# testingautomated-usi/simple-tip

Measured on AMD Instinct MI355X. Metric: inputs_per_sec_prioritized, higher is better.
Workload: dtype bf16; 1 GPU; model=cifar10_resnet20, global_batch=20480, parallelism=dp1, train_ats=50000, at_width=4096, input_residency=hbm, scorers=gini+softmax-family+dsa+pc-lsa

## Files before the change

### simple_tip_amd/ops/hip/bindings.cpp

```cpp

#include <torch/extension.h>

#include <ATen/hip/HIPContext.h>
#include <c10/hip/HIPStream.h>
#include <hip/hip_runtime.h>

#include <vector>

void launch_rownorm(const float*, int, int, float*, hipStream_t);
void launch_pairwise_full(const float*, const float*, const float*,
                          const float*, int, int, int, float*, hipStream_t);
void launch_pairwise_rowmin(const float*, const float*, const float*,
                            const float*, int, int, int, float*, int*, float*,
                            int64_t*, hipStream_t);
void launch_pairwise_kde(const float*, const float*, const float*,
                         const float*, int, int, int, float2*, float*,
                         hipStream_t);
void launch_grouped_rowmin(const float*, const float*, const float*,
                           const float*, const int*, const int*, int, int,
                           int, int, float*, int*, float*, int64_t*,
                           hipStream_t);
void launch_grouped_kde(const float*, const float*, const float*,
                        const float*, const int*, const int*, int, int, int,
                        int, float2*, float*, hipStream_t);
void launch_grouped_rowmin_bf16(const short*, const short*, const float*,
                                const float*, const int*, const int*, int,
                                int, int, int, float*, int*, float*,
                                int64_t*, hipStream_t);
void launch_grouped_kde_bf16(const short*, const short*, const float*,
                             const float*, const int*, const int*, int, int,
                             int, int, float2*, float*, hipStream_t);
void launch_profile(int, const float*, const unsigned char*, const float*,
                    const float*, float, int, int, int, int,
                    unsigned long long*, long long*, hipStream_t);
void launch_popcount(const unsigned long long*, int, int, long long*,
                     hipStream_t);
void launch_tknc(const float*, int, int, int, int, int, unsigned long long*,
                 hipStream_t);
void launch_bucketize(const double*, const double*, int, int, int,
                      unsigned long long*, hipStream_t);
void launch_cam_greedy_coop(const unsigned long long*, int, int,
                            unsigned long long, unsigned char*,
                            unsigned long long*, long long*, int*, long long*,
                            int*, int*, int*, hipStream_t);
void launch_softmax_scores(const float*, int, int, float*, float*, float*,
                           float*, hipStream_t);
void launch_mfma_probe(const short*, const short*, float*, hipStream_t);
void launch_resblock(int, int, const short*, short*, const short*,
                     const float*, const short*, const float*, hipStream_t);
void launch_downblock(int, int, const short*, short*, const short*,
                      const float*, const short*, const float*, const short*,
                      const float*, hipStream_t);
void launch_stem(int, const short*, short*, const short*, const float*,
                 hipStream_t);
void launch_stage1(int, const float*, short*, const void* const*, hipStream_t);
void launch_stage2(int, const short*, short*, const void* const*, hipStream_t);
void launch_stage3(int, const short*, short*, float*, const void* const*,
                   hipStream_t);
void launch_mc_dropout_votes(const float*, const float*, const float*, int,
                             int, int, int, uint32_t, float, uint32_t,
                             uint32_t, uint32_t, int*, hipStream_t);
void launch_mc_dropout_stats(const float*, const float*, const float*, int,
                             int, int, int, uint32_t, float, uint32_t,
                             uint32_t, uint32_t, int*, float*, float*,
                             hipStream_t);
int segment_plan_max_classes();
void launch_segment_plan(const int64_t*, int, int, int, int*, int*, int*,
                         hipStream_t);
void launch_rownorm_bf16(const short*, int, int, const int*, float*,
                         hipStream_t);
int grouped_whiten_max_features();
void launch_grouped_whiten_bf16(const short*, int, int, const int*, const int*,
                                const int*, int, const int*, const short*, int,
                                int, int, int, short*, hipStream_t);
void launch_grouped_rowmin_plan(const short*, int, const short*, const float*,
                                const float*, const int*, const int*,
                                const int*, const float*, int, int, int, int,
                                float*, int*, float*, float*, int*,
                                hipStream_t);
void launch_grouped_kde_plan(const short*, const short*, const float*,
                             const float*, const int*, const int*, const int*,
                             int, const int*, const float*, int, int, int, int,
                             float2*, float*, hipStream_t);
void launch_grouped_center(const void*, bool, int, int, const int*, const int*,
                           const int*, int, int, const float*, int, float*,
                           hipStream_t);
int grouped_gauss_max_slots();
void launch_grouped_gauss_plan(const float*, const float*, const int*,
                               const int*, const int*, int, const float*, int,
                               int, int, int, float*, float*, hipStream_t);
int mc_dropout_max_grid(int, int);
int mc_dropout_rows_per_block();
int mc_dropout_max_classes();
int mc_dropout_max_features();

namespace {

hipStream_t cur_stream() {
  return c10::hip::getCurrentHIPStream().stream();
}

void check_f32_2d(const torch::Tensor& t, const char* name) {
  TORCH_CHECK(t.is_cuda(), name, " must be on GPU");
  TORCH_CHECK(t.dtype() == torch::kFloat32, name, " must be fp32");
  TORCH_CHECK(t.dim() == 2 && t.is_contiguous(), name,
              " must be 2D contiguous");
}

constexpr int kBN = 128;

torch::Tensor rownorm(torch::Tensor x) {
  check_f32_2d(x, "x");
  auto out = torch::empty({x.size(0)}, x.options());
  launch_rownorm(x.data_ptr<float>(), x.size(0), x.size(1),
                 out.data_ptr<float>(), cur_stream());
  return out;
}

torch::Tensor pairwise_sqdist(torch::Tensor a, torch::Tensor b) {
  check_f32_2d(a, "a");
  check_f32_2d(b, "b");
  TORCH_CHECK(a.size(1) == b.size(1), "feature dims differ");
  const int m = a.size(0), n = b.size(0), k = a.size(1);
  auto an = rownorm(a);
  auto bn = rownorm(b);
  auto out = torch::empty({m, n}, a.options());
  launch_pairwise_full(a.data_ptr<float>(), b.data_ptr<float>(),
                       an.data_ptr<float>(), bn.data_ptr<float>(), m, n, k,
                       out.data_ptr<float>(), cur_stream());
  return out;
}

std::vector<torch::Tensor> rowmin_l2(torch::Tensor a, torch::Tensor b,
                                     c10::optional<torch::Tensor> bnorm) {
  check_f32_2d(a, "a");
  check_f32_2d(b, "b");
  TORCH_CHECK(a.size(1) == b.size(1), "feature dims differ");
  TORCH_CHECK(b.size(0) > 0, "rowmin_l2 against empty set");
  const int m = a.size(0), n = b.size(0), k = a.size(1);
  const int jb = (n + kBN - 1) / kBN;
  auto an = rownorm(a);
  auto bn = bnorm.has_value() ? bnorm.value() : rownorm(b);
  auto pval = torch::empty({jb, m}, a.options());
  auto pidx = torch::empty({jb, m}, a.options().dtype(torch::kInt32));
  auto dist = torch::empty({m}, a.options());
  auto idx = torch::empty({m}, a.options().dtype(torch::kInt64));
  launch_pairwise_rowmin(a.data_ptr<float>(), b.data_ptr<float>(),
                         an.data_ptr<float>(), bn.data_ptr<float>(), m, n, k,
                         pval.data_ptr<float>(), pidx.data_ptr<int>(),
                         dist.data_ptr<float>(), idx.data_ptr<int64_t>(),
                         cur_stream());
  return {dist, idx};
}

std::vector<torch::Tensor> grouped_rowmin(
    torch::Tensor testS, torch::Tensor trainS, torch::Tensor tseg,
    torch::Tensor nseg, torch::Tensor bnorm, int64_t jb_max) {
  check_f32_2d(testS, "testS");
  check_f32_2d(trainS, "trainS");
  TORCH_CHECK(tseg.is_cuda() && tseg.dtype() == torch::kInt32);
  TORCH_CHECK(nseg.is_cuda() && nseg.dtype() == torch::kInt32);
  const int bp = testS.size(0), k = testS.size(1);
  const int nclasses = tseg.size(0) - 1;
  auto an = rownorm(testS);
  auto pval = torch::empty({jb_max, bp}, testS.options());
  auto pidx = torch::empty({jb_max, bp}, testS.options().dtype(torch::kInt32));
  auto dist = torch::empty({bp}, testS.options());
  auto idx = torch::empty({bp}, testS.options().dtype(torch::kInt64));
  launch_grouped_rowmin(
      testS.data_ptr<float>(), trainS.data_ptr<float>(), an.data_ptr<float>(),
      bnorm.data_ptr<float>(), tseg.data_ptr<int>(), nseg.data_ptr<int>(),
      nclasses, bp, k, jb_max, pval.data_ptr<float>(), pidx.data_ptr<int>(),
      dist.data_ptr<float>(), idx.data_ptr<int64_t>(), cur_stream());
  return {dist, idx};
}

torch::Tensor grouped_kde(torch::Tensor testWS, torch::Tensor trainWS,
                          torch::Tensor tseg, torch::Tensor nseg,
                          torch::Tensor bnorm, int64_t jb_max) {
  check_f32_2d(testWS, "testWS");
  check_f32_2d(trainWS, "trainWS");
  const int bp = testWS.size(0), k = testWS.size(1);
  const int nclasses = tseg.size(0) - 1;
  auto an = rownorm(testWS);
// ... 497 lines not shown
    const torch::Tensor& b = take();
    TORCH_CHECK(b.is_cuda() && b.dtype() == torch::kFloat32 &&
                    b.is_contiguous() && b.numel() == n,
                "fp32 stage parameter has the wrong type or size");
    ptrs.push_back(b.data_ptr<float>());
  }
  void res(int64_t c) {
    conv(9 * c, c);
    conv(9 * c, c);
  }
  void down(int64_t c) {
    conv(9 * c, 2 * c);
    conv(18 * c, 2 * c);
    conv(c, 2 * c);
  }
  const void* const* done() {
    TORCH_CHECK(next == t.size(), "too many stage parameters");
    return ptrs.data();
  }
};

void check_plane(const torch::Tensor& x, int64_t elems) {
  TORCH_CHECK(x.dim() == 2 && x.size(1) == elems, "x must be [B, ", elems, "]");
}

torch::Tensor resnet_stage1(torch::Tensor x,
                            std::vector<torch::Tensor> params) {
  TORCH_CHECK(x.is_cuda() && x.dtype() == torch::kFloat32 &&
                  x.is_contiguous() && x.dim() == 4 && x.size(1) == 32 &&
                  x.size(2) == 32 && x.size(3) == 3,
              "x must be a contiguous fp32 [B, 32, 32, 3] GPU tensor");
  TORCH_CHECK(reinterpret_cast<uintptr_t>(x.data_ptr()) % 16 == 0,
              "x must be 16-byte aligned");
  StageParams p(params);
  p.conv(9 * 8, 16);
  for (int i = 0; i < 3; ++i) p.res(16);
  p.down(16);
  const void* const* ptrs = p.done();
  const int batch = x.size(0);
  auto out = torch::empty({batch, 16 * 16 * 32},
                          x.options().dtype(torch::kBFloat16));
  if (batch > 0)
    launch_stage1(batch, x.data_ptr<float>(),
                  const_cast<short*>(bf16_ptr(out)), ptrs, cur_stream());
  return out;
}

torch::Tensor resnet_stage2(torch::Tensor x,
                            std::vector<torch::Tensor> params) {
  check_plane(x, 16 * 16 * 32);
  StageParams p(params);
  for (int i = 0; i < 2; ++i) p.res(32);
  p.down(32);
  const void* const* ptrs = p.done();
  const int batch = x.size(0);
  auto out = torch::empty({batch, 8 * 8 * 64}, x.options());
  if (batch > 0)
    launch_stage2(batch, bf16_ptr(x), const_cast<short*>(bf16_ptr(out)), ptrs,
                  cur_stream());
  return out;
}

std::vector<torch::Tensor> resnet_stage3(torch::Tensor x,
                                         std::vector<torch::Tensor> params) {
  check_plane(x, 8 * 8 * 64);
  StageParams p(params);
  for (int i = 0; i < 2; ++i) p.res(64);
  p.f32(10 * 64);
  p.f32(10);
  const void* const* ptrs = p.done();
  const int batch = x.size(0);
  auto ats = torch::empty_like(x);
  auto logits = torch::empty({batch, 10}, x.options().dtype(torch::kFloat32));
  if (batch > 0)
    launch_stage3(batch, bf16_ptr(x), const_cast<short*>(bf16_ptr(ats)),
                  logits.data_ptr<float>(), ptrs, cur_stream());
  return {ats, logits};
}


static void mc_dropout_check(const torch::Tensor& feats,
                             const torch::Tensor& weight,
                             const torch::Tensor& bias, int64_t thresh,
                             int64_t num_samples, int64_t row_offset) {
  check_f32_2d(feats, "feats");
  check_f32_2d(weight, "weight");
  TORCH_CHECK(bias.is_cuda() && bias.dtype() == torch::kFloat32 &&
                  bias.dim() == 1 && bias.is_contiguous(),
              "bias must be a contiguous 1D fp32 GPU tensor");
  const int64_t n = feats.size(0), d = feats.size(1), c = weight.size(0);
  TORCH_CHECK(weight.size(1) == d, "weight must be [C, D]");
  TORCH_CHECK(bias.size(0) == c, "bias must be [C]");
  TORCH_CHECK(c >= 1 && c <= mc_dropout_max_classes() && d >= 1 &&
                  d <= mc_dropout_max_features(),
              "mc_dropout_votes envelope is C <= ", mc_dropout_max_classes(),
              ", D <= ", mc_dropout_max_features());
  TORCH_CHECK(num_samples >= 1 && num_samples <= 65535, "bad num_samples");
  TORCH_CHECK(thresh >= 0 && thresh <= 0xFFFFFFFFll, "bad threshold");
  TORCH_CHECK(n <= 0x7FFFFFFFll && row_offset >= 0 &&
                  row_offset + n <= 0x100000000ll,
              "rows must satisfy row_offset + N <= 2^32");
}

torch::Tensor mc_dropout_votes(torch::Tensor feats, torch::Tensor weight,
                               torch::Tensor bias, int64_t thresh,
                               double scale, int64_t num_samples,
                               int64_t seed_lo, int64_t seed_hi,
                               int64_t row_offset) {
  mc_dropout_check(feats, weight, bias, thresh, num_samples, row_offset);
  const int64_t n = feats.size(0), d = feats.size(1), c = weight.size(0);
  auto votes = torch::empty({n, c}, feats.options().dtype(torch::kInt32));
  if (n == 0) return votes;
  launch_mc_dropout_votes(
      feats.data_ptr<float>(), weight.data_ptr<float>(),
      bias.data_ptr<float>(), (int)n, (int)d, (int)c, (int)num_samples,
      (uint32_t)thresh, (float)scale, (uint32_t)seed_lo, (uint32_t)seed_hi,
      (uint32_t)row_offset, votes.data_ptr<int>(), cur_stream());
  return votes;
}

std::vector<torch::Tensor> mc_dropout_stats(
    torch::Tensor feats, torch::Tensor weight, torch::Tensor bias,
    int64_t thresh, double scale, int64_t num_samples, int64_t seed_lo,
    int64_t seed_hi, int64_t row_offset) {
  mc_dropout_check(feats, weight, bias, thresh, num_samples, row_offset);
  const int64_t n = feats.size(0), d = feats.size(1), c = weight.size(0);
  auto votes = torch::empty({n, c}, feats.options().dtype(torch::kInt32));
  auto mean_probs = torch::empty({n, c}, feats.options());
  auto mean_entropy = torch::empty({n}, feats.options());
  if (n == 0) return {votes, mean_probs, mean_entropy};
  launch_mc_dropout_stats(
      feats.data_ptr<float>(), weight.data_ptr<float>(),
      bias.data_ptr<float>(), (int)n, (int)d, (int)c, (int)num_samples,
      (uint32_t)thresh, (float)scale, (uint32_t)seed_lo, (uint32_t)seed_hi,
      (uint32_t)row_offset, votes.data_ptr<int>(),
      mean_probs.data_ptr<float>(), mean_entropy.data_ptr<float>(),
      cur_stream());
  return {votes, mean_probs, mean_entropy};
}

}

PYBIND11_MODULE(TORCH_EXTENSION_NAME, m) {
  m.doc() = "simple_tip_amd HIP/CDNA4 kernels (gfx950)";
  m.def("rownorm", &rownorm);
  m.def("pairwise_sqdist", &pairwise_sqdist);
  m.def("rowmin_l2", &rowmin_l2, py::arg("a"), py::arg("b"),
        py::arg("bnorm") = py::none());
  m.def("kde_logsumexp", &kde_logsumexp);
  m.def("grouped_rowmin", &grouped_rowmin);
  m.def("grouped_kde", &grouped_kde);
  m.def("grouped_rowmin_bf16", &grouped_rowmin_bf16);
  m.def("grouped_kde_bf16", &grouped_kde_bf16);
  m.def("segment_plan", &segment_plan);
  m.def("segment_plan_out", &segment_plan_out);
  m.def("segment_plan_rows", &segment_plan_rows);
  m.def("rownorm_bf16_out", &rownorm_bf16_out, py::arg("x"), py::arg("out"),
        py::arg("tseg") = py::none());
  m.def("grouped_whiten_bf16", &grouped_whiten_bf16);
  m.def("grouped_whiten_max_features", &grouped_whiten_max_features);
  m.def("grouped_rowmin_plan", &grouped_rowmin_plan);
  m.def("grouped_kde_plan", &grouped_kde_plan);
  m.def("grouped_gauss_plan", &grouped_gauss_plan, py::arg("x"),
        py::arg("tseg"), py::arg("rowmap"), py::arg("comp_off"),
        py::arg("means"), py::arg("mats"), py::arg("logc"), py::arg("slots"),
        py::arg("dc"), py::arg("pquad"), py::arg("out"));
  m.def("grouped_gauss_max_slots", &grouped_gauss_max_slots);
  m.def("profile", &profile);
  m.def("pack_bits", &pack_bits);
  m.def("popcount_rows", &popcount_rows);
  m.def("tknc_layer", &tknc_layer);
  m.def("bucketize", &bucketize);
  m.def("cam_greedy", &cam_greedy);
  m.def("softmax_scores", &softmax_scores);
  m.def("levenshtein_matrix", &levenshtein_matrix);
  m.def("mfma_probe", &mfma_probe);
  m.def("resnet_block", &resnet_block);
  m.def("resnet_down", &resnet_down);
  m.def("resnet_stem", &resnet_stem);
  m.def("resnet_stage1", &resnet_stage1);
  m.def("resnet_stage2", &resnet_stage2);
  m.def("resnet_stage3", &resnet_stage3);
  m.def("mc_dropout_votes", &mc_dropout_votes);
  m.def("mc_dropout_stats", &mc_dropout_stats);
  m.def("mc_dropout_max_grid", &mc_dropout_max_grid);
  m.def("mc_dropout_rows_per_block", &mc_dropout_rows_per_block);
  m.def("mc_dropout_max_classes", &mc_dropout_max_classes);
  m.def("mc_dropout_max_features", &mc_dropout_max_features);
}
```

### simple_tip_amd/ops/hip/pairwise.hip

```cpp

#include "tip_common.h"

#include <cfloat>
#include <cmath>

using f32x16 = __attribute__((__vector_size__(16 * sizeof(float)))) float;

constexpr int BM = 128;
constexpr int BN = 128;
constexpr int BK = 32;
constexpr int LDS_PAD = 4;

enum Epilogue { EPI_FULL = 0, EPI_ROWMIN = 1, EPI_KDE = 2, EPI_QUAD = 3 };


struct StageRegs {
  float4 v[4];
};

TIP_DEV StageRegs stage_load(
    const float* __restrict__ src, int rows, int K, int row0, int k0) {
  StageRegs sr;
  const int t = threadIdx.x;
  const int r = t >> 1;
// ... 255 lines not shown
    const float* __restrict__ anorm,
    const float* __restrict__ bnorm,
    const int* __restrict__ tseg,
    const int* __restrict__ nseg,
    int nclasses, int Bp, int K,
    float* __restrict__ pmin_val,
    int* __restrict__ pmin_idx,
    float2* __restrict__ pkde) {
  __shared__ float lds[2 * BK * (BM + LDS_PAD)];
  __shared__ float red_v[BM][2];
  __shared__ int red_i[BM][2];
  __shared__ float red_s[BM][2];

  const int bj = blockIdx.x;
  const int row0 = blockIdx.y * BM;
  if (row0 >= Bp) return;
  const int cls = class_of_row(tseg, nclasses, row0);
  const int ncol1 = nseg[cls + 1];
  const int col0 = nseg[cls] + bj * BN;
  if (col0 >= ncol1) return;

  const TileAcc acc = tile_mainloop_f32(A, Bp, B, ncol1, K, row0, col0, lds,
                                        lds + BK * (BM + LDS_PAD));
  tile_epilogue_f32<EPI>(acc, anorm, bnorm, row0, Bp, col0, ncol1, Bp, bj,
                         red_v, red_i, red_s, nullptr, pmin_val, pmin_idx,
                         pkde);
}


__launch_bounds__(256, 2) __global__ void grouped_quad_kernel(
    const float* __restrict__ dc,
    const float* __restrict__ mats,
    const int* __restrict__ tseg,
    const int* __restrict__ comp_off,
    int ngroups, int Bp, int D,
    float* __restrict__ pquad) {
  __shared__ float lds[2 * BK * (BM + LDS_PAD)];
  __shared__ float red_v[BM][2];

  const int bj = blockIdx.x;
  const int row0 = blockIdx.y * BM;
  const int s = blockIdx.z;
  if (row0 >= Bp || row0 >= tseg[ngroups]) return;
  const int g = class_of_row(tseg, ngroups, row0);
  if (s >= comp_off[g + 1] - comp_off[g]) return;
  const int mrow0 = (comp_off[g] + s) * D;
  const float* a = dc + (int64_t)s * Bp * D;

  const TileAcc acc =
      tile_mainloop_f32(a, Bp, mats, mrow0 + D, D, row0, mrow0 + bj * BN, lds,
                        lds + BK * (BM + LDS_PAD));
  tile_epilogue_quad(acc, a, D, row0, Bp, bj * BN, Bp, s * gridDim.x + bj,
                     red_v, pquad);
}

constexpr int QUAD_MAX_SLOTS = 8;

__global__ void grouped_gauss_final_kernel(
    const float* __restrict__ pquad, const int* __restrict__ tseg,
    const int* __restrict__ comp_off, int ngroups, int Bp, int jb,
    const int* __restrict__ rowmap, int out_rows,
    const float* __restrict__ logc,
    int mode, float* __restrict__ out) {
  const int i = blockIdx.x * blockDim.x + threadIdx.x;
  if (i >= Bp || i >= tseg[ngroups]) return;
  const int src = rowmap[i];
  if (src < 0 || src >= out_rows) return;
  const int g = class_of_row(tseg, ngroups, i);
  const int c0 = comp_off[g];
  int ncomp = comp_off[g + 1] - c0;
  if (ncomp > QUAD_MAX_SLOTS) ncomp = QUAD_MAX_SLOTS;
  if (ncomp <= 0) {
    out[src] = INFINITY;
    return;
  }
  float t[QUAD_MAX_SLOTS];
  float tmax = -INFINITY;
#pragma unroll
  for (int s = 0; s < QUAD_MAX_SLOTS; ++s) {
    t[s] = -INFINITY;
    if (s < ncomp) {
      float q = 0.f;
      for (int b = 0; b < jb; ++b) q += pquad[((int64_t)s * jb + b) * Bp + i];
      t[s] = (mode == 0) ? q : (logc[c0 + s] - 0.5f * q);
      tmax = fmaxf(tmax, t[s]);
    }
  }
  if (mode == 0) {
    out[src] = t[0];
    return;
  }
  if (!(tmax > -INFINITY && tmax < INFINITY)) {
    out[src] = (tmax == -INFINITY) ? INFINITY : -tmax;
    return;
  }
  float sum = 0.f;
#pragma unroll
  for (int s = 0; s < QUAD_MAX_SLOTS; ++s)
    if (s < ncomp) sum += expf(t[s] - tmax);
  out[src] = -(tmax + logf(sum));
}


using bf16x8 = __attribute__((ext_vector_type(8))) short;
using f32x4b = __attribute__((ext_vector_type(4))) float;

constexpr int BBK = 32;
#ifndef TIP_BROW
#define TIP_BROW 40
#endif
constexpr int BROW = TIP_BROW;

struct BStage {
  bf16x8 v[2];
};

TIP_DEV BStage bstage_load_row(const short* __restrict__ src, int grow,
                               bool ok, int K, int k0) {
  BStage s;
  const int kq = (threadIdx.x & 1) * 16;
  const bf16x8 zero = {0, 0, 0, 0, 0, 0, 0, 0};
#pragma unroll
  for (int h = 0; h < 2; ++h) {
    const int gk = k0 + kq + h * 8;
    if (ok && gk + 7 < K) {
      s.v[h] = *reinterpret_cast<const bf16x8*>(&src[(int64_t)grow * K + gk]);
    } else if (ok) {
      bf16x8 tmp = zero;
      for (int e = 0; e < 8; ++e)
        if (gk + e < K) tmp[e] = src[(int64_t)grow * K + gk + e];
      s.v[h] = tmp;
    } else {
      s.v[h] = zero;
    }
  }
  return s;
}

TIP_DEV BStage bstage_load(const short* __restrict__ src, int rows, int K,
                           int row0, int k0) {
  const int grow = row0 + (threadIdx.x >> 1);
  return bstage_load_row(src, grow, grow < rows, K, k0);
}

TIP_DEV void bstage_write(short* lds, const BStage& s) {
  const int t = threadIdx.x;
  const int r = t >> 1;
  const int kq = (t & 1) * 16;
  *reinterpret_cast<bf16x8*>(&lds[r * BROW + kq]) = s.v[0];
  *reinterpret_cast<bf16x8*>(&lds[r * BROW + kq + 8]) = s.v[1];
}

template <int EPI, bool GATHER>
__launch_bounds__(256, 2) __global__ void grouped_pairwise_bf16_kernel(
    const short* __restrict__ A,
    const short* __restrict__ B,
    const float* __restrict__ anorm,
    const float* __restrict__ bnorm,
    const int* __restrict__ tseg, const int* __restrict__ nseg,
    const int* __restrict__ rowmap,
    int a_rows,
    int nclasses, int Bp, int K,
    float* __restrict__ pmin_val, int* __restrict__ pmin_idx,
    float2* __restrict__ pkde) {
  __shared__ short As[128 * BROW];
  __shared__ short Bs[128 * BROW];
  __shared__ float red_v[BM][2];
  __shared__ int red_i[BM][2];
  __shared__ float red_s[BM][2];

  const int bi = blockIdx.y;
  const int bj = blockIdx.x;
  const int row0 = bi * BM;
  if (row0 >= tseg[nclasses]) return;
  const int cls = class_of_row(tseg, nclasses, row0);
  const int ncol0 = nseg[cls], ncol1 = nseg[cls + 1];
  const int col0 = ncol0 + bj * BN;
  if (col0 >= ncol1) return;

  const int lane = lane_id();
  const int wid = wave_id();
  const int wr = wid >> 1;
  const int wc = wid & 1;
  const int fj = lane & 15;
  const int fg = lane >> 4;

  int arow = row0 + (threadIdx.x >> 1);
  bool arow_ok = arow < Bp;
  if (GATHER) {
    arow = arow_ok ? rowmap[arow] : -1;
    arow_ok = arow >= 0 && arow < a_rows;
  }

  f32x4b acc[4][4] = {};
  BStage ra = bstage_load_row(A, arow, arow_ok, K, 0);
  BStage rb = bstage_load(B, ncol1, K, col0, 0);
  bstage_write(As, ra);
  bstage_write(Bs, rb);
  __syncthreads();
  for (int k0 = 0; k0 < K; k0 += BBK) {
    const bool has_next = (k0 + BBK) < K;
    if (has_next) {
      ra = bstage_load_row(A, arow, arow_ok, K, k0 + BBK);
      rb = bstage_load(B, ncol1, K, col0, k0 + BBK);
    }
    bf16x8 af[4], bf[4];
#pragma unroll
    for (int t = 0; t < 4; ++t) {
      const int i = wr * 64 + t * 16 + fj;
      const int j = wc * 64 + t * 16 + fj;
      af[t] = *reinterpret_cast<const bf16x8*>(&As[i * BROW + fg * 8]);
      bf[t] = *reinterpret_cast<const bf16x8*>(&Bs[j * BROW + fg * 8]);
    }
#pragma unroll
    for (int tr = 0; tr < 4; ++tr)
#pragma unroll
      for (int tc = 0; tc < 4; ++tc)
        acc[tr][tc] = __builtin_amdgcn_mfma_f32_16x16x32_bf16(
            af[tr], bf[tc], acc[tr][tc], 0, 0, 0);
    __syncthreads();
    if (has_next) {
      bstage_write(As, ra);
      bstage_write(Bs, rb);
    }
    __syncthreads();
  }

#pragma unroll
  for (int tr = 0; tr < 4; ++tr) {
#pragma unroll
    for (int reg = 0; reg < 4; ++reg) {
      const int row_local = wr * 64 + tr * 16 + fg * 4 + reg;
      const int gi = row0 + row_local;
      float an;
      if (GATHER) {
        const int src = rowmap[gi];
        an = (src >= 0 && src < a_rows) ? anorm[src] : 0.f;
      } else {
        an = anorm[gi];
      }
      MinIdx mi{FLT_MAX, 0x7fffffff};
      float dvals[4];
#pragma unroll
      for (int tc = 0; tc < 4; ++tc) {
        const int gj = col0 + wc * 64 + tc * 16 + fj;
        float d;
        if (gj < ncol1) {
          d = fmaxf(an + bnorm[gj] - 2.f * acc[tr][tc][reg], 0.f);
        } else {
          d = FLT_MAX;
        }
        dvals[tc] = d;
        mi = min_idx_combine(mi, MinIdx{d, gj});
      }
      for (int off = 8; off >= 1; off >>= 1) {
        MinIdx o;
        o.v = __shfl_xor(mi.v, off);
        o.i = __shfl_xor(mi.i, off);
        mi = min_idx_combine(mi, o);
      }
      if (EPI == EPI_ROWMIN) {
        if (fj == 0) {
          red_v[row_local][wc] = mi.v;
          red_i[row_local][wc] = mi.i;
        }
      } else {
        const float tmax = (mi.v == FLT_MAX) ? -FLT_MAX : -0.5f * mi.v;
        float s = 0.f;
#pragma unroll
        for (int tc = 0; tc < 4; ++tc)
          if (dvals[tc] != FLT_MAX) s += __expf(-0.5f * dvals[tc] - tmax);
        for (int off = 8; off >= 1; off >>= 1) s += __shfl_xor(s, off);
        if (fj == 0) {
          red_v[row_local][wc] = tmax;
          red_s[row_local][wc] = s;
        }
      }
    }
  }
  __syncthreads();
  merge_halves_store<EPI>(red_v, red_i, red_s, row0, Bp, Bp, bj, pmin_val,
                          pmin_idx, pkde);
}


TIP_DEV MinIdx fold_rowmin(const float* __restrict__ pval,
                           const int* __restrict__ pidx, int jcount,
                           int stride, int i) {
  MinIdx best{FLT_MAX, 0x7fffffff};
  for (int b = 0; b < jcount; ++b)
    best = min_idx_combine(best, MinIdx{pval[(int64_t)b * stride + i],
                                        pidx[(int64_t)b * stride + i]});
  return best;
}

TIP_DEV float fold_kde(const float2* __restrict__ pkde, int jcount, int stride,
                       int i) {
  float mm = -FLT_MAX, ss = 0.f;
  for (int b = 0; b < jcount; ++b) {
    const float2 p = pkde[(int64_t)b * stride + i];
    if (p.y <= 0.f) continue;
    if (p.x > mm) {
      ss = p.y + ((ss > 0.f) ? ss * __expf(mm - p.x) : 0.f);
      mm = p.x;
    } else {
      ss += p.y * __expf(p.x - mm);
    }
  }
  return (ss > 0.f) ? (mm + __logf(ss)) : -FLT_MAX;
}

TIP_DEV int class_jcount(const int* __restrict__ nseg, int cls) {
  return (nseg[cls + 1] - nseg[cls] + BN - 1) / BN;
}

__global__ void rowmin_combine_kernel(
    const float* __restrict__ pval, const int* __restrict__ pidx, int jblocks,
    int M, float* __restrict__ out_dist, int64_t* __restrict__ out_idx) {
  const int i = blockIdx.x * blockDim.x + threadIdx.x;
  if (i >= M) return;
  const MinIdx best = fold_rowmin(pval, pidx, jblocks, M, i);
  out_dist[i] = sqrtf(best.v);
  out_idx[i] = best.i;
}

__global__ void kde_combine_kernel(
    const float2* __restrict__ pkde, int jblocks, int M,
    float* __restrict__ out_lse) {
  const int i = blockIdx.x * blockDim.x + threadIdx.x;
  if (i >= M) return;
  out_lse[i] = fold_kde(pkde, jblocks, M, i);
}

__global__ void grouped_rowmin_combine_kernel(
    const float* __restrict__ pval, const int* __restrict__ pidx,
    const int* __restrict__ tseg, const int* __restrict__ nseg, int nclasses,
    int Bp, float* __restrict__ out_dist, int64_t* __restrict__ out_idx) {
  const int i = blockIdx.x * blockDim.x + threadIdx.x;
  if (i >= Bp) return;
  const int jcount = class_jcount(nseg, class_of_row(tseg, nclasses, i));
  const MinIdx best = fold_rowmin(pval, pidx, jcount, Bp, i);
  if (jcount == 0) {
    out_dist[i] = FLT_MAX;
    out_idx[i] = -1;
  } else {
    out_dist[i] = sqrtf(best.v);
    out_idx[i] = best.i;
  }
}

__global__ void grouped_kde_combine_kernel(
    const float2* __restrict__ pkde, const int* __restrict__ tseg,
    const int* __restrict__ nseg, int nclasses, int Bp,
    float* __restrict__ out_lse) {
  const int i = blockIdx.x * blockDim.x + threadIdx.x;
  if (i >= Bp) return;
  const int jcount = class_jcount(nseg, class_of_row(tseg, nclasses, i));
  out_lse[i] = fold_kde(pkde, jcount, Bp, i);
}

__global__ void grouped_rowmin_final_kernel(
    const float* __restrict__ pval, const int* __restrict__ pidx,
    const int* __restrict__ tseg, const int* __restrict__ nseg, int nclasses,
    int Bp, const int* __restrict__ rowmap, int out_rows,
    const float* __restrict__ btable, float* __restrict__ out_dsa,
    float* __restrict__ out_dist, int* __restrict__ out_idx) {
  const int i = blockIdx.x * blockDim.x + threadIdx.x;
  if (i >= Bp || i >= tseg[nclasses]) return;
  const int src = rowmap[i];
  if (src < 0 || src >= out_rows) return;
  const int jcount = class_jcount(nseg, class_of_row(tseg, nclasses, i));
  const MinIdx best = fold_rowmin(pval, pidx, jcount, Bp, i);
  if (jcount == 0) {
    out_dsa[src] = INFINITY;
    out_dist[src] = FLT_MAX;
    out_idx[src] = -1;
  } else if ((unsigned)best.i >= (unsigned)nseg[nclasses]) {
    out_dsa[src] = NAN;
    out_dist[src] = NAN;
    out_idx[src] = -1;
  } else {
    const float dist = sqrtf(best.v);
    out_dsa[src] = dist / btable[best.i];
    out_dist[src] = dist;
    out_idx[src] = best.i;
  }
}

__global__ void grouped_kde_final_kernel(
    const float2* __restrict__ pkde, const int* __restrict__ tseg,
    const int* __restrict__ nseg, int nclasses, int Bp,
    const int* __restrict__ rowmap, int out_rows,
    const int* __restrict__ cls_fused,
    const float* __restrict__ cls_const,
    float* __restrict__ out_lsa) {
  const int i = blockIdx.x * blockDim.x + threadIdx.x;
  if (i >= Bp || i >= tseg[nclasses]) return;
  const int src = rowmap[i];
  if (src < 0 || src >= out_rows) return;
  const int cls = class_of_row(tseg, nclasses, i);
  if (!cls_fused[cls]) {
    out_lsa[src] = cls_const[cls];
    return;
  }
  const float lse = fold_kde(pkde, class_jcount(nseg, cls), Bp, i);
  out_lsa[src] = -(lse + cls_const[cls]);
}

__global__ void rownorm_kernel(
    const float* __restrict__ X, int rows, int K, float* __restrict__ out) {
  const int row = blockIdx.x * (blockDim.x / WAVE) + wave_id();
  if (row >= rows) return;
  const float* p = X + (int64_t)row * K;
  float s = 0.f;
  for (int k = lane_id(); k < K; k += WAVE) {
    const float v = p[k];
    s += v * v;
  }
  for (int off = 32; off >= 1; off >>= 1) s += __shfl_xor(s, off);
  if (lane_id() == 0) out[row] = s;
}


void launch_rownorm(const float* x, int rows, int k, float* out, hipStream_t s) {
  const int wpb = 4;
  rownorm_kernel<<<ceil_div(rows, wpb), wpb * WAVE, 0, s>>>(x, rows, k, out);
}

void launch_pairwise_full(const float* a, const float* b, const float* an,
                          const float* bn, int m, int n, int k, float* out,
                          hipStream_t s) {
  dim3 grid(ceil_div(n, BN), ceil_div(m, BM));
  pairwise_kernel<EPI_FULL><<<grid, 256, 0, s>>>(
      a, b, an, bn, m, n, k, out, nullptr, nullptr, nullptr);
}

void launch_pairwise_rowmin(const float* a, const float* b, const float* an,
                            const float* bn, int m, int n, int k,
                            float* pval, int* pidx, float* out_dist,
                            int64_t* out_idx, hipStream_t s) {
  const int jb = ceil_div(n, BN);
  dim3 grid(jb, ceil_div(m, BM));
  pairwise_kernel<EPI_ROWMIN><<<grid, 256, 0, s>>>(
      a, b, an, bn, m, n, k, nullptr, pval, pidx, nullptr);
  rowmin_combine_kernel<<<ceil_div(m, 256), 256, 0, s>>>(
      pval, pidx, jb, m, out_dist, out_idx);
}

void launch_pairwise_kde(const float* a, const float* b, const float* an,
                         const float* bn, int m, int n, int k, float2* pkde,
                         float* out_lse, hipStream_t s) {
  const int jb = ceil_div(n, BN);
  dim3 grid(jb, ceil_div(m, BM));
  pairwise_kernel<EPI_KDE><<<grid, 256, 0, s>>>(
      a, b, an, bn, m, n, k, nullptr, nullptr, nullptr, pkde);
  kde_combine_kernel<<<ceil_div(m, 256), 256, 0, s>>>(pkde, jb, m, out_lse);
}

void launch_grouped_rowmin(const float* a, const float* b, const float* an,
                           const float* bn, const int* tseg, const int* nseg,
                           int nclasses, int bp, int k, int jb_max,
                           float* pval, int* pidx, float* out_dist,
                           int64_t* out_idx, hipStream_t s) {
  dim3 grid(jb_max, ceil_div(bp, BM));
  grouped_pairwise_kernel<EPI_ROWMIN><<<grid, 256, 0, s>>>(
      a, b, an, bn, tseg, nseg, nclasses, bp, k, pval, pidx, nullptr);
  grouped_rowmin_combine_kernel<<<ceil_div(bp, 256), 256, 0, s>>>(
      pval, pidx, tseg, nseg, nclasses, bp, out_dist, out_idx);
}

void launch_grouped_kde(const float* a, const float* b, const float* an,
                        const float* bn, const int* tseg, const int* nseg,
                        int nclasses, int bp, int k, int jb_max, float2* pkde,
                        float* out_lse, hipStream_t s) {
  dim3 grid(jb_max, ceil_div(bp, BM));
  grouped_pairwise_kernel<EPI_KDE><<<grid, 256, 0, s>>>(
      a, b, an, bn, tseg, nseg, nclasses, bp, k, nullptr, nullptr, pkde);
  grouped_kde_combine_kernel<<<ceil_div(bp, 256), 256, 0, s>>>(
      pkde, tseg, nseg, nclasses, bp, out_lse);
}

void launch_grouped_rowmin_bf16(const short* a, const short* b,
                                const float* an, const float* bn,
                                const int* tseg, const int* nseg,
                                int nclasses, int bp, int k, int jb_max,
                                float* pval, int* pidx, float* out_dist,
                                int64_t* out_idx, hipStream_t s) {
  dim3 grid(jb_max, ceil_div(bp, BM));
  grouped_pairwise_bf16_kernel<EPI_ROWMIN, false><<<grid, 256, 0, s>>>(
      a, b, an, bn, tseg, nseg, nullptr, 0, nclasses, bp, k, pval, pidx,
      nullptr);
  grouped_rowmin_combine_kernel<<<ceil_div(bp, 256), 256, 0, s>>>(
      pval, pidx, tseg, nseg, nclasses, bp, out_dist, out_idx);
}

void launch_grouped_kde_bf16(const short* a, const short* b, const float* an,
                             const float* bn, const int* tseg,
                             const int* nseg, int nclasses, int bp, int k,
                             int jb_max, float2* pkde, float* out_lse,
                             hipStream_t s) {
  dim3 grid(jb_max, ceil_div(bp, BM));
  grouped_pairwise_bf16_kernel<EPI_KDE, false><<<grid, 256, 0, s>>>(
      a, b, an, bn, tseg, nseg, nullptr, 0, nclasses, bp, k, nullptr, nullptr,
      pkde);
  grouped_kde_combine_kernel<<<ceil_div(bp, 256), 256, 0, s>>>(
      pkde, tseg, nseg, nclasses, bp, out_lse);
}

void launch_grouped_rowmin_plan(const short* a, int a_rows, const short* b,
                                const float* an, const float* bn,
                                const int* tseg, const int* nseg,
                                const int* rowmap, const float* btable,
                                int nclasses, int bp, int k, int jb_max,
                                float* pval, int* pidx, float* out_dsa,
                                float* out_dist, int* out_idx, hipStream_t s) {
  dim3 grid(jb_max, ceil_div(bp, BM));
  grouped_pairwise_bf16_kernel<EPI_ROWMIN, true><<<grid, 256, 0, s>>>(
      a, b, an, bn, tseg, nseg, rowmap, a_rows, nclasses, bp, k, pval, pidx,
      nullptr);
  grouped_rowmin_final_kernel<<<ceil_div(bp, 256), 256, 0, s>>>(
      pval, pidx, tseg, nseg, nclasses, bp, rowmap, a_rows, btable, out_dsa,
      out_dist, out_idx);
}

int grouped_gauss_max_slots() { return QUAD_MAX_SLOTS; }

void launch_grouped_gauss_plan(const float* dc, const float* mats,
                               const int* tseg, const int* comp_off,
                               const int* rowmap, int out_rows,
                               const float* logc, int ngroups, int bp, int d,
                               int slots, float* pquad, float* out,
                               hipStream_t s) {
  const int jb = ceil_div(d, BN);
  dim3 grid(jb, ceil_div(bp, BM), slots);
  grouped_quad_kernel<<<grid, 256, 0, s>>>(dc, mats, tseg, comp_off, ngroups,
                                           bp, d, pquad);
  grouped_gauss_final_kernel<<<ceil_div(bp, 256), 256, 0, s>>>(
      pquad, tseg, comp_off, ngroups, bp, jb, rowmap, out_rows, logc,
      logc != nullptr ? 1 : 0, out);
}

void launch_grouped_kde_plan(const short* a, const short* b, const float* an,
                             const float* bn, const int* tseg,
                             const int* nseg, const int* rowmap, int out_rows,
                             const int* cls_fused, const float* cls_const,
                             int nclasses, int bp, int k, int jb_max,
                             float2* pkde, float* out_lsa, hipStream_t s) {
  dim3 grid(jb_max, ceil_div(bp, BM));
  grouped_pairwise_bf16_kernel<EPI_KDE, false><<<grid, 256, 0, s>>>(
      a, b, an, bn, tseg, nseg, nullptr, 0, nclasses, bp, k, nullptr, nullptr,
      pkde);
  grouped_kde_final_kernel<<<ceil_div(bp, 256), 256, 0, s>>>(
      pkde, tseg, nseg, nclasses, bp, rowmap, out_rows, cls_fused, cls_const,
      out_lsa);
}
```

Baseline: 5.276 million inputs/s.

## Add double-buffered direct-to-LDS pipelined bf16 rowmin kernel with XCD-aware block remap

Adds a new rowmin kernel for the DSA bf16 pairwise-distance GEMM. It loads A and B tiles straight into LDS via global_load_lds, double-buffers BK=64 tiles so the next stage's loads overlap the current MFMAs, and uses an XOR-swizzled layout to avoid bank conflicts. Block ids are remapped so neighbouring tiles land on the same XCD, which should improve L2 reuse. The epilogue is factored out and shared. The new path is used whenever K is a multiple of 64 and pointers are 16-byte aligned, and out-of-range rows read from a zero buffer. This costs 64KB of LDS per block, which may reduce occupancy.

```diff
diff --git a/simple_tip_amd/ops/hip/bindings.cpp b/simple_tip_amd/ops/hip/bindings.cpp
--- a/simple_tip_amd/ops/hip/bindings.cpp
+++ b/simple_tip_amd/ops/hip/bindings.cpp
@@ -30,6 +30,10 @@
 void launch_grouped_kde_bf16(const short*, const short*, const float*,
                              const float*, const int*, const int*, int, int,
                              int, int, float2*, float*, hipStream_t);
+void rowmin_bf16_force_generic(bool);
+int64_t rowmin_bf16_pipelined_launches();
+int rowmin_bf16_pipeline_bk();
+int rowmin_bf16_pipeline_nbuf();
 void launch_profile(int, const float*, const unsigned char*, const float*,
                     const float*, float, int, int, int, int,
                     unsigned long long*, long long*, hipStream_t);
@@ -833,6 +837,10 @@
   m.def("grouped_kde", &grouped_kde);
   m.def("grouped_rowmin_bf16", &grouped_rowmin_bf16);
   m.def("grouped_kde_bf16", &grouped_kde_bf16);
+  m.def("rowmin_bf16_force_generic", &rowmin_bf16_force_generic);
+  m.def("rowmin_bf16_pipelined_launches", &rowmin_bf16_pipelined_launches);
+  m.def("rowmin_bf16_pipeline_bk", &rowmin_bf16_pipeline_bk);
+  m.def("rowmin_bf16_pipeline_nbuf", &rowmin_bf16_pipeline_nbuf);
   m.def("segment_plan", &segment_plan);
   m.def("segment_plan_out", &segment_plan_out);
   m.def("segment_plan_rows", &segment_plan_rows);
diff --git a/simple_tip_amd/ops/hip/pairwise.hip b/simple_tip_amd/ops/hip/pairwise.hip
--- a/simple_tip_amd/ops/hip/pairwise.hip
+++ b/simple_tip_amd/ops/hip/pairwise.hip
@@ -431,6 +431,15 @@
 }
 
 template <int EPI, bool GATHER>
+TIP_DEV void bf16_tile_epilogue(
+    const f32x4b (&acc)[4][4], const float* __restrict__ anorm,
+    const float* __restrict__ bnorm, const int* __restrict__ rowmap,
+    int a_rows, int row0, int col0, int ncol1, int Bp, int bj,
+    float (*red_v)[2], int (*red_i)[2], float (*red_s)[2],
+    float* __restrict__ pmin_val, int* __restrict__ pmin_idx,
+    float2* __restrict__ pkde);
+
+template <int EPI, bool GATHER>
 __launch_bounds__(256, 2) __global__ void grouped_pairwise_bf16_kernel(
     const short* __restrict__ A,
     const short* __restrict__ B,
@@ -504,6 +513,25 @@
     }
     __syncthreads();
   }
+
+  bf16_tile_epilogue<EPI, GATHER>(acc, anorm, bnorm, rowmap, a_rows, row0,
+                                  col0, ncol1, Bp, bj, red_v, red_i, red_s,
+                                  pmin_val, pmin_idx, pkde);
+}
+
+template <int EPI, bool GATHER>
+TIP_DEV void bf16_tile_epilogue(
+    const f32x4b (&acc)[4][4], const float* __restrict__ anorm,
+    const float* __restrict__ bnorm, const int* __restrict__ rowmap,
+    int a_rows, int row0, int col0, int ncol1, int Bp, int bj,
+    float (*red_v)[2], int (*red_i)[2], float (*red_s)[2],
+    float* __restrict__ pmin_val, int* __restrict__ pmin_idx,
+    float2* __restrict__ pkde) {
+  const int lane = lane_id();
+  const int wr = wave_id() >> 1;
+  const int wc = wave_id() & 1;
+  const int fj = lane & 15;
+  const int fg = lane >> 4;
 
 #pragma unroll
   for (int tr = 0; tr < 4; ++tr) {
@@ -563,6 +591,131 @@
 }
 
 
+constexpr int PBK = 64;
+constexpr int PNBUF = 2;
+constexpr int PTILE = 128 * PBK;
+
+static __device__ __attribute__((aligned(128))) short g_zero_units[PBK];
+
+#ifndef TIP_ROWMIN_XCD
+#define TIP_ROWMIN_XCD 1
+#endif
+
+using lds_ptr_t = __attribute__((address_space(3))) void*;
+using glb_ptr_t = const __attribute__((address_space(1))) void*;
+
+template <bool GATHER>
+__launch_bounds__(256, 2) __global__ void grouped_rowmin_bf16_pipe_kernel(
+    const short* __restrict__ A,
+    const short* __restrict__ B,
+    const float* __restrict__ anorm, const float* __restrict__ bnorm,
+    const int* __restrict__ tseg, const int* __restrict__ nseg,
+    const int* __restrict__ rowmap,
+    int a_rows,
+    int nclasses, int Bp, int K,
+    float* __restrict__ pmin_val, int* __restrict__ pmin_idx) {
+  __shared__ __attribute__((aligned(16))) short lds[PNBUF * 2 * PTILE];
+
+  int bi = blockIdx.y, bj = blockIdx.x;
+  if (TIP_ROWMIN_XCD) {
+    const int nwg = gridDim.x * gridDim.y;
+    const int id = blockIdx.y * gridDim.x + blockIdx.x;
+    const int q = nwg / 8, r = nwg % 8;
+    const int xcd = id % 8, pos = id / 8;
+    const int newid =
+        (xcd < r ? xcd * (q + 1) : r * (q + 1) + (xcd - r) * q) + pos;
+    bi = newid / gridDim.x;
+    bj = newid % gridDim.x;
+  }
+  const int row0 = bi * BM;
+  if (row0 >= tseg[nclasses]) return;
+  const int cls = class_of_row(tseg, nclasses, row0);
+  const int ncol0 = nseg[cls], ncol1 = nseg[cls + 1];
+  const int col0 = ncol0 + bj * BN;
+  if (col0 >= ncol1) return;
+
+  const int t = threadIdx.x;
+  const int lane = lane_id();
+  const int wid = wave_id();
+  const int wr = wid >> 1;
+  const int wc = wid & 1;
+  const int fj = lane & 15;
+  const int fg = lane >> 4;
+
+  const int sunit = (t & 7) ^ ((t >> 3) & 7);
+  const short* asrc[4];
+  const short* bsrc[4];
+  int astep[4], bstep[4];
+#pragma unroll
+  for (int q = 0; q < 4; ++q) {
+    const int r = q * 32 + (t >> 3);
+    int arow = row0 + r;
+    bool aok = arow < Bp;
+    if (GATHER) {
+      arow = aok ? rowmap[arow] : -1;
+      aok = arow >= 0 && arow < a_rows;
+    }
+    asrc[q] = (aok ? A + (int64_t)arow * K : g_zero_units) + sunit * 8;
+    astep[q] = aok ? PBK : 0;
+    const int brow = col0 + r;
+    const bool bok = brow < ncol1;
+    bsrc[q] = (bok ? B + (int64_t)brow * K : g_zero_units) + sunit * 8;
+    bstep[q] = bok ? PBK : 0;
+  }
+  auto stage = [&](int buf) {
+    short* dst = lds + buf * 2 * PTILE + wid * 64 * 8;
+#pragma unroll
+    for (int q = 0; q < 4; ++q) {
+      __builtin_amdgcn_global_load_lds((glb_ptr_t)asrc[q],
+                                       (lds_ptr_t)(dst + q * 256 * 8), 16, 0,
+                                       0);
+      __builtin_amdgcn_global_load_lds(
+          (glb_ptr_t)bsrc[q], (lds_ptr_t)(dst + PTILE + q * 256 * 8), 16, 0, 0);
+      asrc[q] += astep[q];
+      bsrc[q] += bstep[q];
+    }
+  };
+
+  const int aoff = (wr * 64 + fj) * PBK;
+  const int boff = PTILE + (wc * 64 + fj) * PBK;
+  const int uoff[2] = {((fg) ^ (fj & 7)) * 8, ((4 + fg) ^ (fj & 7)) * 8};
+
+  f32x4b acc[4][4] = {};
+  const int ntiles = K / PBK;
+  stage(0);
+  for (int kt = 0; kt < ntiles; ++kt) {
+    asm volatile("s_waitcnt vmcnt(0)" ::: "memory");
+    __syncthreads();
+    if (kt + 1 < ntiles) stage((kt + 1) & 1);
+    const short* cur = lds + (kt & 1) * 2 * PTILE;
+#pragma unroll
+    for (int s = 0; s < 2; ++s) {
+      bf16x8 af[4], bf[4];
+#pragma unroll
+      for (int f = 0; f < 4; ++f) {
+        af[f] = *reinterpret_cast<const bf16x8*>(
+            &cur[aoff + f * 16 * PBK + uoff[s]]);
+        bf[f] = *reinterpret_cast<const bf16x8*>(
+            &cur[boff + f * 16 * PBK + uoff[s]]);
+      }
+#pragma unroll
+      for (int tr = 0; tr < 4; ++tr)
+#pragma unroll
+        for (int tc = 0; tc < 4; ++tc)
+          acc[tr][tc] = __builtin_amdgcn_mfma_f32_16x16x32_bf16(
+              af[tr], bf[tc], acc[tr][tc], 0, 0, 0);
+    }
+  }
+
+  __syncthreads();
+  float(*red_v)[2] = reinterpret_cast<float(*)[2]>(lds);
+  int(*red_i)[2] = reinterpret_cast<int(*)[2]>(lds + BM * 2 * 2);
+  bf16_tile_epilogue<EPI_ROWMIN, GATHER>(
+      acc, anorm, bnorm, rowmap, a_rows, row0, col0, ncol1, Bp, bj, red_v,
+      red_i, nullptr, pmin_val, pmin_idx, nullptr);
+}
+
+
 TIP_DEV MinIdx fold_rowmin(const float* __restrict__ pval,
                            const int* __restrict__ pidx, int jcount,
                            int stride, int i) {
@@ -759,6 +912,22 @@
       pkde, tseg, nseg, nclasses, bp, out_lse);
 }
 
+static bool g_rowmin_force_generic = false;
+static int64_t g_rowmin_pipelined_launches = 0;
+
+void rowmin_bf16_force_generic(bool on) { g_rowmin_force_generic = on; }
+int64_t rowmin_bf16_pipelined_launches() { return g_rowmin_pipelined_launches; }
+int rowmin_bf16_pipeline_bk() { return PBK; }
+int rowmin_bf16_pipeline_nbuf() { return PNBUF; }
+
+static bool rowmin_bf16_use_pipeline(const short* a, const short* b, int k) {
+  const bool ok = !g_rowmin_force_generic && k > 0 && k % PBK == 0 &&
+                  ((reinterpret_cast<uintptr_t>(a) |
+                    reinterpret_cast<uintptr_t>(b)) & 15) == 0;
+  if (ok) ++g_rowmin_pipelined_launches;
+  return ok;
+}
+
 void launch_grouped_rowmin_bf16(const short* a, const short* b,
                                 const float* an, const float* bn,
                                 const int* tseg, const int* nseg,
@@ -766,9 +935,13 @@
                                 float* pval, int* pidx, float* out_dist,
                                 int64_t* out_idx, hipStream_t s) {
   dim3 grid(jb_max, ceil_div(bp, BM));
-  grouped_pairwise_bf16_kernel<EPI_ROWMIN, false><<<grid, 256, 0, s>>>(
-      a, b, an, bn, tseg, nseg, nullptr, 0, nclasses, bp, k, pval, pidx,
-      nullptr);
+  if (rowmin_bf16_use_pipeline(a, b, k))
+    grouped_rowmin_bf16_pipe_kernel<false><<<grid, 256, 0, s>>>(
+        a, b, an, bn, tseg, nseg, nullptr, 0, nclasses, bp, k, pval, pidx);
+  else
+    grouped_pairwise_bf16_kernel<EPI_ROWMIN, false><<<grid, 256, 0, s>>>(
+        a, b, an, bn, tseg, nseg, nullptr, 0, nclasses, bp, k, pval, pidx,
+        nullptr);
   grouped_rowmin_combine_kernel<<<ceil_div(bp, 256), 256, 0, s>>>(
       pval, pidx, tseg, nseg, nclasses, bp, out_dist, out_idx);
 }
@@ -794,9 +967,13 @@
                                 float* pval, int* pidx, float* out_dsa,
                                 float* out_dist, int* out_idx, hipStream_t s) {
   dim3 grid(jb_max, ceil_div(bp, BM));
-  grouped_pairwise_bf16_kernel<EPI_ROWMIN, true><<<grid, 256, 0, s>>>(
-      a, b, an, bn, tseg, nseg, rowmap, a_rows, nclasses, bp, k, pval, pidx,
-      nullptr);
+  if (rowmin_bf16_use_pipeline(a, b, k))
+    grouped_rowmin_bf16_pipe_kernel<true><<<grid, 256, 0, s>>>(
+        a, b, an, bn, tseg, nseg, rowmap, a_rows, nclasses, bp, k, pval, pidx);
+  else
+    grouped_pairwise_bf16_kernel<EPI_ROWMIN, true><<<grid, 256, 0, s>>>(
+        a, b, an, bn, tseg, nseg, rowmap, a_rows, nclasses, bp, k, pval, pidx,
+        nullptr);
   grouped_rowmin_final_kernel<<<ceil_div(bp, 256), 256, 0, s>>>(
       pval, pidx, tseg, nseg, nclasses, bp, rowmap, a_rows, btable, out_dsa,
       out_dist, out_idx);
```

Result: faster. 5.560 million inputs/s, median of 6 (+5.4%).
